# pascalPost/turbomesh

Measured on AMD Instinct MI355X. Metric: nodes smoothed/sec (elliptic sweeps, 4096^2 blocks) + achieved HBM GB/s, higher is better.
Workload: dtype f64

## Files before the change

turbomesh_amd/csrc/tm_kernels.hip:

```cpp
#include "tm_kernels.h"
#include "tm_devutil.hpp"
#include "tm_refmath.h"
#include <cstdlib>
#include <type_traits>

namespace tmh {

__device__ __forceinline__ double lane_prev(double edge, double v) {
    int2 o = __builtin_bit_cast(int2, edge), s = __builtin_bit_cast(int2, v), r;
    r.x = __builtin_amdgcn_update_dpp(o.x, s.x, 0x138 , 0xf, 0xf, false);
    r.y = __builtin_amdgcn_update_dpp(o.y, s.y, 0x138, 0xf, 0xf, false);
    return __builtin_bit_cast(double, r);
}
__device__ __forceinline__ double lane_next(double edge, double v) {
    int2 o = __builtin_bit_cast(int2, edge), s = __builtin_bit_cast(int2, v), r;
    r.x = __builtin_amdgcn_update_dpp(o.x, s.x, 0x130 , 0xf, 0xf, false);
    r.y = __builtin_amdgcn_update_dpp(o.y, s.y, 0x130, 0xf, 0xf, false);
    return __builtin_bit_cast(double, r);
}
__device__ __forceinline__ double2 lane_prev(double2 edge, double2 v) { return make_double2(lane_prev(edge.x, v.x), lane_prev(edge.y, v.y)); }
__device__ __forceinline__ double2 lane_next(double2 edge, double2 v) { return make_double2(lane_next(edge.x, v.x), lane_next(edge.y, v.y)); }

__device__ __forceinline__ double2 lane_prev0(double2 v) {
    int4 s = __builtin_bit_cast(int4, v), r;
// ... 12 lines not shown
    return __builtin_bit_cast(double2, r);
}

enum { S_I_J = 0, S_IP1_J, S_IM1_J, S_I_JP1, S_I_JM1, S_IP1_JP1, S_IP1_JM1, S_IM1_JP1, S_IM1_JM1 };

template <bool HAS_PQ>
__device__ __forceinline__ void stencil_coefs(double2 im1_j, double2 ip1_j, double2 i_jm1, double2 i_jp1, double P, double Q,
                                              double (&c)[9]) {
    const double x_xi = 0.5 * (ip1_j.x - im1_j.x);
    const double x_eta = 0.5 * (i_jp1.x - i_jm1.x);
    const double y_xi = 0.5 * (ip1_j.y - im1_j.y);
    const double y_eta = 0.5 * (i_jp1.y - i_jm1.y);
    const double g22 = x_eta * x_eta + y_eta * y_eta;
    const double g12 = x_xi * x_eta + y_xi * y_eta;
    const double g11 = x_xi * x_xi + y_xi * y_xi;
    c[S_I_J] = -2.0 * g22 - 2.0 * g11;
    if (HAS_PQ) {
        c[S_IP1_J] = g22 * (1 + 0.5 * P);
        c[S_IM1_J] = g22 * (1 - 0.5 * P);
        c[S_I_JP1] = g11 * (1 + 0.5 * Q);
        c[S_I_JM1] = g11 * (1 - 0.5 * Q);
    } else {
        c[S_IP1_J] = g22;
        c[S_IM1_J] = g22;
        c[S_I_JP1] = g11;
        c[S_I_JM1] = g11;
    }
    c[S_IP1_JP1] = -0.5 * g12;
    c[S_IP1_JM1] = 0.5 * g12;
    c[S_IM1_JP1] = 0.5 * g12;
    c[S_IM1_JM1] = -0.5 * g12;
}

template <int MODE>
__device__ __forceinline__ double row_out(double sum, double rhs, double diag, double in_self, double omega) {
    if (MODE == MODE_RAW) return sum;
    const double dinv = (diag == 0.0) ? 1.0 : 1.0 / diag;
    if (MODE == MODE_SCALED) return sum * dinv;
    const double res = rhs * dinv - sum * dinv;
    if (MODE == MODE_RESID) return res;
    return in_self + omega * res;
}

template <int DOT>
__device__ __forceinline__ void accumulate(double (&acc)[MAX_PARTIALS], double2 in_self, double2 out, double2 aux) {
    if (DOT == DOT_AUX) {
        acc[0] += aux.x * out.x;
        acc[1] += aux.y * out.y;
    } else if (DOT == DOT_AUX2) {
        acc[0] += aux.x * out.x;
        acc[1] += aux.y * out.y;
        acc[2] += out.x * out.x;
        acc[3] += out.y * out.y;
    } else if (DOT == DOT_IN) {
        acc[0] += in_self.x * out.x;
        acc[1] += in_self.y * out.y;
        acc[2] += out.x * out.x;
        acc[3] += out.y * out.y;
    } else if (DOT == DOT_IN_SS) {
        acc[0] += in_self.x * out.x;
        acc[1] += in_self.y * out.y;
        acc[2] += out.x * out.x;
        acc[3] += out.y * out.y;
        acc[4] += in_self.x * in_self.x;
        acc[5] += in_self.y * in_self.y;
    } else if (DOT == DOT_B2) {
        acc[0] += in_self.x * out.x;
        acc[1] += in_self.y * out.y;
        acc[2] += out.x * out.x;
        acc[3] += out.y * out.y;
        acc[4] += aux.x * in_self.x;
        acc[5] += aux.y * in_self.y;
        acc[6] += aux.x * out.x;
        acc[7] += aux.y * out.y;
    } else if (DOT == DOT_OUT2) {
        acc[0] += out.x * out.x;
        acc[1] += out.y * out.y;
    } else if (DOT == DOT_DELTA) {
        acc[0] = fma(aux.x, aux.x, acc[0]);
        acc[1] = fma(aux.y, aux.y, acc[1]);
    }
}

__device__ __forceinline__ double recip_diag(double D, double m2D) {
    const bool plain = (D >= 0x1p-700) && (D <= 0x1p700);
    if (__builtin_amdgcn_ballot_w64(!plain) == 0) {
        const double nd = -m2D;
        const double r0 = __builtin_amdgcn_rcp(m2D);
        const double e0 = fma(nd, r0, 1.0);
        const double r1 = fma(r0, e0, r0);
        const double e1 = fma(nd, r1, 1.0);
        const double r2 = fma(r1, e1, r1);
        const double e2 = fma(nd, r2, 1.0);
        return fma(e2, r2, r2);
    }
    return (D == 0.0) ? 0.25 : 1.0 / m2D;
}

template <int MODE, bool HAS_PQ, bool UNIT_OMEGA = false>
__device__ __forceinline__ double2 winslow_row(double2 m_c, double2 e_m, double2 c_c, double2 e_c, double2 h_c, double2 p_c, double2 e_p, double2 dxi,
                                               double2 det, double P, double Q, double omega, double2& delta) {
    const double G11 = fma(dxi.x, dxi.x, dxi.y * dxi.y);
    const double G22 = fma(det.x, det.x, det.y * det.y);
    const double G12 = fma(dxi.x, det.x, dxi.y * det.y);
    const double D = G11 + G22;
    const double m2D = -2.0 * D;
    const double mhG12 = -0.5 * G12;
    double ax = p_c.x + m_c.x, ay = p_c.y + m_c.y;
    double bx = h_c.x, by = h_c.y;
    if (HAS_PQ) {
        const double hP = 0.5 * P, hQ = 0.5 * Q;
        ax = fma(hP, p_c.x - m_c.x, ax);
        ay = fma(hP, p_c.y - m_c.y, ay);
        bx = fma(hQ, e_c.x, bx);
        by = fma(hQ, e_c.y, by);
    }
    const double kx = e_p.x - e_m.x;
    const double ky = e_p.y - e_m.y;
    double sx = G22 * ax, sy = G22 * ay;
    sx = fma(G11, bx, sx);
    sy = fma(G11, by, sy);
    if (MODE == MODE_RELAX && (UNIT_OMEGA || omega == 1.0)) {
        const double qx = fma(mhG12, kx, sx), qy = fma(mhG12, ky, sy);
        const bool plain = (D >= 0x1p-700) && (D <= 0x1p700);
        double2 xn;
        if (__builtin_amdgcn_ballot_w64(!plain) == 0) {
            const double nd = -m2D;
            const double r0 = __builtin_amdgcn_rcp(m2D);
            const double e0 = fma(nd, r0, 1.0);
            const double r1 = fma(r0, e0, r0);
            const double e1 = fma(nd, r1, 1.0);
            const double r2 = fma(r1, e1, r1);
            const double e2 = fma(nd, r2, 1.0);
            const double r = fma(e2, r2, r2);
            xn = make_double2(-(qx * r), -(qy * r));
        } else {
            const double r = 1.0 / m2D;
            xn = (D == 0.0) ? c_c : make_double2(-(qx * r), -(qy * r));
        }
        delta = make_double2(xn.x - c_c.x, xn.y - c_c.y);
        return xn;
    }
    sx = fma(m2D, c_c.x, sx);
    sy = fma(m2D, c_c.y, sy);
    sx = fma(mhG12, kx, sx);
    sy = fma(mhG12, ky, sy);
    if (MODE == MODE_RAW) return make_double2(0.25 * sx, 0.25 * sy);
    const double rinv = recip_diag(D, m2D);
    const double tx = sx * rinv, ty = sy * rinv;
    if (MODE == MODE_SCALED) return make_double2(tx, ty);
    if (MODE == MODE_RESID) return make_double2(-tx, -ty);
    delta = UNIT_OMEGA ? make_double2(-tx, -ty) : make_double2(omega * (-tx), omega * (-ty));
    return make_double2(c_c.x + delta.x, c_c.y + delta.y);
}

__device__ __forceinline__ double2 sub2(double2 a, double2 b) { return make_double2(a.x - b.x, a.y - b.y); }
__device__ __forceinline__ double2 add2(double2 a, double2 b) { return make_double2(a.x + b.x, a.y + b.y); }

template <int NT>
__device__ __forceinline__ const KrylovScalars* lazy_scalars(const LazyScalars& L);

static bool g_rows_forced = false;
static int g_rows_per_chunk = 18;
static int g_unroll = 6;
static int g_nt = 1;

constexpr unsigned OOB_VOFFSET = 0x80000000u;
typedef int v4i32 __attribute__((ext_vector_type(4)));

typedef double d2v __attribute__((ext_vector_type(2)));
__device__ __forceinline__ void store_nt(double2* dst, double2 v) {
    d2v o;
    o.x = v.x;
    o.y = v.y;
    __builtin_nontemporal_store(o, reinterpret_cast<d2v*>(dst));
}

struct VirtualR {
    double2 s, rn, pn;
};
__device__ __forceinline__ VirtualR virtual_r(double2 x, double2 y, double2 z, double2 w, double2 va, double2 vb, double2 vc) {
    VirtualR o;
    o.s = make_double2(x.x - va.x * y.x, x.y - va.y * y.y);
    o.rn = make_double2(o.s.x - vb.x * z.x, o.s.y - vb.y * z.y);
    o.pn = make_double2(o.rn.x + vc.x * (w.x - vb.x * y.x), o.rn.y + vc.y * (w.y - vb.y * y.y));
    return o;
}
template <int VK>
__device__ __forceinline__ double2 virtual_vec(double2 x, double2 y, double2 z, double2 va, double2 vb) {
    if (VK == VK_S || VK == VK_S2) return make_double2(x.x - va.x * y.x, x.y - va.y * y.y);
    if (VK == VK_P) return make_double2(x.x + va.x * (y.x - vb.x * z.x), x.y + va.y * (y.y - vb.y * z.y));
    return x;
}

__device__ __forceinline__ double2 load_nt(const double2* src);

template <int MODE, int DOT, bool FIELD, bool HAS_PQ, int U, bool NT, int VK = VK_NONE, bool OV = false>
__device__ __forceinline__ void apply_tile(const ApplyBlock& a, int RI, int nSG, int nRC, int bid, double2 va = make_double2(0.0, 0.0),
                                           double2 vb = make_double2(0.0, 0.0), double2 vc = make_double2(0.0, 0.0)) {
    static_assert(U % 3 == 0, "the 3-row window rotates by renaming: the row group must be a multiple of 3");
    const int lane = threadIdx.x & 63;
    const int wave = threadIdx.x >> 6;
    const int total = nSG * nRC;
    const int q = total >> 3, rem = total & 7, xcd = bid & 7, k = bid >> 3;
    const int logical = (xcd < rem) ? xcd * (q + 1) + k : rem * (q + 1) + (xcd - rem) * q + k;
    const int rc = logical / nSG;
    const int sg = logical - rc * nSG;

    const int ni = a.ni, nj = a.nj;
    const int j0 = (sg * 4 + wave) * (OV ? 62 : 64);
    const int j = j0 + lane;
    const int jc = min(j, nj - 1);
    const bool edge_lane = !OV && ((lane == 0) || (lane == 63));
    const int hcol = (lane == 0) ? max(j0 - 1, 0) : min(j0 + 64, nj - 1);
    const bool valid_col = (j >= 1) && (j <= nj - 2) && (!OV || (lane >= 1 && lane <= 62));
    const bool full_wave = !OV && (j0 >= 1) && (j0 + 63 <= nj - 2);
    const int i0 = 1 + rc * RI;
    const int i1 = min(i0 + RI, ni - 1);

    double acc[MAX_PARTIALS] = {0.0, 0.0, 0.0, 0.0};
    if ((OV ? (j0 + 1 <= nj - 2) : (j0 < nj)) && i0 < i1) {
// ... 200 lines not shown
                    } else {
                        *dst = o;
                    }
                    if (VK == VK_P) store_nt(a.pout + static_cast<size_t>(row) * nj + j, Wc[C]);
                    accumulate<DOT>(acc, Wc[C], o, (DOT == DOT_AUX || DOT == DOT_AUX2 || DOT == DOT_B2) ? g.auxv[u] : ((DOT == DOT_DELTA) ? delta : o));
                }
                if (!FIELD) Xdet = sub2(lane_next(g.xph[u], g.xpc[u]), lane_prev(g.xph[u], g.xpc[u]));
            }
        };

        int ib = i0;
        if (full_wave) {
            for (; ib + U <= i1; ib += U) {
                Group g;
                load_group(ib, g);
                compute_group(ib, g, std::false_type{});
            }
        }
        for (; ib < i1; ib += U) {
            Group g;
            load_group(ib, g);
            compute_group(ib, g, std::true_type{});
        }
    }
    if ((MODE == MODE_DIAG_NOSTORE || MODE == MODE_DIAG_MATH) && acc[0] + acc[1] == 123.456) a.out[0] = make_double2(acc[0], acc[1]);
    if (DOT != DOT_NONE) block_partials<256, (VK == VK_R ? 4 : dot_columns(DOT))>(acc, a.partials + static_cast<size_t>(bid) * MAX_PARTIALS);
}

template <int MODE, int DOT, bool FIELD, bool HAS_PQ, int U, bool NT>
__global__ __launch_bounds__(256) void k_apply(ApplyBlock a, int RI, int nSG, int nRC) {
    apply_tile<MODE, DOT, FIELD, HAS_PQ, U, NT>(a, RI, nSG, nRC, blockIdx.x);
}

template <int MODE, int DOT, bool FIELD, bool HAS_PQ, int U, bool NT>
__global__ __launch_bounds__(256) void k_apply_batch(ApplyBatch B) {
    int k = 0;
#pragma unroll
    for (int q = 1; q < APPLY_BATCH_MAX; ++q)
        if (q < B.n && static_cast<int>(blockIdx.x) >= B.start[q]) k = q;
    apply_tile<MODE, DOT, FIELD, HAS_PQ, U, NT>(B.b[k], B.RI[k], B.nSG[k], B.nRC[k], static_cast<int>(blockIdx.x) - B.start[k]);
}


template <bool HAS_PQ>
__global__ __launch_bounds__(256) void k_apply_prolong_smooth(ApplyBlock a, int RI, int nSG, int nRC) {
    apply_tile<MODE_MG_SMOOTH, DOT_NONE, false, HAS_PQ, 3, true, VK_PRO>(a, RI, nSG, nRC, blockIdx.x);
}
static inline int rows_per_chunk(int ni, int nj, int rows);
hipError_t launch_mg_prolong_smooth(const ApplyBlock& a0, const MgPair& g, hipStream_t st) {
    if (a0.ni < 3 || a0.nj < 3) return hipSuccess;
    ApplyBlock a = a0;
    a.mg_nic = g.nic;
    a.mg_njc = g.njc;
    a.mg_ci = g.ci;
    a.mg_cj = g.cj;
    const int RI = rows_per_chunk(a.ni, a.nj, a.rows);
    const int nSG = (a.nj + 255) / 256;
    const int nRC = (a.ni - 2 + RI - 1) / RI;
    const dim3 grid(nSG * nRC), block(256);
    if (a.pq) hipLaunchKernelGGL(k_apply_prolong_smooth<true>, grid, block, 0, st, a, RI, nSG, nRC);
    else hipLaunchKernelGGL(k_apply_prolong_smooth<false>, grid, block, 0, st, a, RI, nSG, nRC);
    return hipGetLastError();
}

struct Relax2Tile {
    int c0, c, i0, i1;
    bool out_lane;
};

#ifndef TM_R2_SAUX
#define TM_R2_SAUX 2
#endif
struct Row3 {
    double2 c, e, h;
};
__device__ __forceinline__ Row3 make_row(double2 c) {
    const double2 l = lane_prev0(c), r = lane_next0(c);
    Row3 w;
    w.c = c;
    w.e = sub2(r, l);
    w.h = add2(r, l);
    return w;
}
template <bool W1>
__device__ __forceinline__ double2 relax_row(const Row3& m, const Row3& c, const Row3& p, double omega, double2& delta) {
    return winslow_row<MODE_RELAX, false, W1>(m.c, m.e, c.c, c.e, c.h, p.c, p.e, sub2(p.c, m.c), c.e, 0.0, 0.0, omega, delta);
}

template <int DOT, int U, int NT, bool W1>
__device__ __forceinline__ void relax2_strip_edge(const Relax2Block& a, const Relax2Tile& t, double (&acc)[MAX_PARTIALS]) {
    const int ni = a.ni, nj = a.nj;
    const int cc = min(max(t.c, 0), nj - 1);
    const double2* in_col = a.in + cc;
    const double2* mid_col = a.mid + cc;
    const double2 zero = make_double2(0.0, 0.0);
    auto load_in = [&](int row) { return in_col[static_cast<size_t>(min(max(row, 0), ni - 1)) * nj]; };
    auto load_mid = [&](int row) { return mid_col[static_cast<size_t>(min(max(row, 0), ni - 1)) * nj]; };
    const bool perim_col = (t.c == 0) || (t.c == nj - 1);
    const bool ring_col = (t.c == 1) || (t.c == nj - 2);
    const int nrows = t.i1 - t.i0;
    const __amdgpu_buffer_rsrc_t out_rsrc = __builtin_amdgcn_make_buffer_rsrc(a.out + static_cast<size_t>(t.i0) * nj, 0, nrows * nj * 16, 0x00020000);
    const __amdgpu_buffer_rsrc_t mid_rsrc = __builtin_amdgcn_make_buffer_rsrc(a.mid + static_cast<size_t>(t.i0) * nj, 0, nrows * nj * 16, 0x00020000);
    const unsigned lane_off = static_cast<unsigned>(cc) * 16u;

    Row3 A[3], S[3];
    double2 pa[U], na[U], pm;
    {
        const double2 a0 = load_in(t.i0 - 2), a1 = load_in(t.i0 - 1);
#pragma unroll
        for (int u = 0; u < U; ++u) pa[u] = load_in(t.i0 + u);
        pm = load_mid(t.i0 - 1);
        A[0] = make_row(a0);
        A[1] = make_row(a1);
        A[2].c = A[2].e = A[2].h = zero;
        S[0] = S[1] = S[2] = A[2];
    }
    const int nsteps = nrows + 2;
    auto group = [&](const int tb) {
#pragma unroll
        for (int u = 0; u < U; ++u) na[u] = load_in(t.i0 + tb + U + u);
#pragma unroll
        for (int u = 0; u < U; ++u) {
            const int A0 = u % 3, A1 = (u + 1) % 3, A2 = (u + 2) % 3;
            const int i = t.i0 - 2 + tb + u;
            const int q = i + 1;
            A[A2] = make_row(pa[u]);
            const double2 pm_now = pm;
            pm = load_mid(q + 1);
            double2 d1 = zero;
            double2 s1 = relax_row<W1>(A[A0], A[A1], A[A2], a.omega, d1);
            const bool perim_row = (q <= 0) || (q >= ni - 1);
            if (perim_row || perim_col) s1 = pm_now;
            const bool ring = t.out_lane && !perim_row && (q >= t.i0) && (q < t.i1) && ((q == 1) || (q == ni - 2) || ring_col);
            __builtin_amdgcn_raw_buffer_store_b128(__builtin_bit_cast(v4i32, s1), mid_rsrc,
                                                   static_cast<int>(ring ? lane_off + static_cast<unsigned>((q - t.i0) * nj * 16) : OOB_VOFFSET), 0, 0);
            S[A2] = make_row(s1);
            double2 d2 = zero;
            const double2 o = relax_row<W1>(S[A0], S[A1], S[A2], a.omega, d2);
            const bool live = t.out_lane && (i >= t.i0) && (i < t.i1);
            __builtin_amdgcn_raw_buffer_store_b128(__builtin_bit_cast(v4i32, o), out_rsrc,
                                                   static_cast<int>(live ? lane_off + static_cast<unsigned>((i - t.i0) * nj * 16) : OOB_VOFFSET), 0, (NT & 1) ? TM_R2_SAUX : 0);
            if (DOT == DOT_DELTA) {
                if (!live) d2 = zero;
                accumulate<DOT_DELTA>(acc, S[A1].c, o, d2);
            }
        }
#pragma unroll
        for (int u = 0; u < U; ++u) pa[u] = na[u];
    };
    group(0);
    for (int tb = U; tb < nsteps; tb += U) group(tb);
}

template <int DOT, int U, int NT, bool W1>
__device__ __forceinline__ void relax2_strip_inside(const Relax2Block& a, const Relax2Tile& t, double (&acc)[MAX_PARTIALS]) {
    const int nj = a.nj;
    const double2* in_col = a.in + t.c;
    const int last_row = t.i1 + 1;
    auto load_in = [&](int row) {
        const double2* src = in_col + static_cast<size_t>(min(row, last_row)) * nj;
        return (NT & 2) ? load_nt(src) : *src;
    };
    const __amdgpu_buffer_rsrc_t out_rsrc =
        __builtin_amdgcn_make_buffer_rsrc(a.out + static_cast<size_t>(t.i0) * nj, 0, (t.i1 - t.i0) * nj * 16, 0x00020000);
    const unsigned voff = t.out_lane ? static_cast<unsigned>(t.c) * 16u : OOB_VOFFSET;

// ... 91 lines not shown
    if (subset == R2_BORDER) {
        logical = a.border[bid];
    } else {
        const int q8 = total >> 3, rem = total & 7, xcd = bid & 7, k8 = bid >> 3;
        logical = (xcd < rem) ? xcd * (q8 + 1) + k8 : rem * (q8 + 1) + (xcd - rem) * q8 + k8;
    }
    const int rc = logical / nSG;
    const int sg = logical - rc * nSG;

    const int ni = a.ni, nj = a.nj;
    Relax2Tile t;
    t.c0 = (sg * 4 + wave) * 60;
    t.c = t.c0 - 2 + lane;
    t.out_lane = (lane >= 2) && (lane <= 61) && (t.c >= 1) && (t.c <= nj - 2);
    relax2_chunk_rows(ni, RI, rc, t.i0, t.i1);

    if (subset != R2_ALL && subset != R2_BORDER) {
        const bool wg_inside = !relax2_tile_is_border(ni, nj, t.i0, t.i1, sg, a.dyn);
        const bool mine = wg_inside && (subset == R2_INSIDE || ((subset == R2_INSIDE_A) == (rc < nRC / 2)));
        if (!mine) return;
    }
    double acc[MAX_PARTIALS] = {0.0, 0.0, 0.0, 0.0};
    if (t.c0 <= nj - 2 && t.i0 < t.i1) {
        const bool inside = (t.c0 - 2 >= 2) && (t.c0 + 61 <= nj - 3) && (t.i0 - 2 >= 2) && (t.i1 + 1 <= ni - 3) && ((t.i1 - t.i0) % U == 0);
        if (inside) relax2_strip_inside<DOT, U, NT, W1>(a, t, acc);
        else relax2_strip_edge<DOT, U, NT, W1>(a, t, acc);
    }
    if (DOT != DOT_NONE) block_partials<256, dot_columns(DOT)>(acc, a.partials + static_cast<size_t>(logical) * MAX_PARTIALS);
}

template <int DOT, int U, int NT, bool W1>
__global__ __launch_bounds__(256) void k_relax2(Relax2Block a, int RI, int nSG, int nRC, int subset) {
    relax2_tile<DOT, U, NT, W1>(a, RI, nSG, nRC, subset, blockIdx.x);
}

__device__ __forceinline__ void spin_until(const uint32_t* counter, uint32_t target, uint32_t* error, long long limit_ticks) {
    if (__hip_atomic_load(error, __ATOMIC_RELAXED, __HIP_MEMORY_SCOPE_AGENT) != 0u) return;
    const long long t0 = wall_clock64();
    unsigned polls = 0;
    while (__hip_atomic_load(counter, __ATOMIC_RELAXED, __HIP_MEMORY_SCOPE_AGENT) < target) {
        __builtin_amdgcn_s_sleep(16);
        ++polls;
        if ((polls & 255u) != 0u) continue;
        if (__hip_atomic_load(error, __ATOMIC_RELAXED, __HIP_MEMORY_SCOPE_AGENT) != 0u) break;
        if (wall_clock64() - t0 > limit_ticks) {
            __hip_atomic_store(error, 1u, __ATOMIC_RELAXED, __HIP_MEMORY_SCOPE_AGENT);
            break;
        }
    }
}
__device__ __forceinline__ void queue_wait_in_kernel(const QueueWait& w) {
    if (threadIdx.x == 0) spin_until(w.counter, w.target, w.error, w.limit_ticks);
    __syncthreads();
    __builtin_amdgcn_fence(__ATOMIC_ACQUIRE, "agent");
}
__device__ __forceinline__ void queue_signal_in_kernel(uint32_t* counter) {
    if (counter && blockIdx.x == 0 && threadIdx.x == 0) __hip_atomic_fetch_add(counter, 1u, __ATOMIC_RELEASE, __HIP_MEMORY_SCOPE_AGENT);
}
template <int DOT, int U, int NT, bool W1>
__global__ __launch_bounds__(256) void k_relax2_waited(Relax2Block a, int RI, int nSG, int nRC, int subset, QueueWait w) {
    queue_wait_in_kernel(w);
    relax2_tile<DOT, U, NT, W1>(a, RI, nSG, nRC, subset, blockIdx.x);
}

template <int DOT, int U, int NT, bool W1>
__global__ __launch_bounds__(256) void k_relax2_batch_waited(Relax2Batch B, int subset, QueueWait w) {
    queue_wait_in_kernel(w);
    int k = 0;
#pragma unroll
    for (int q = 1; q < APPLY_BATCH_MAX; ++q)
        if (q < B.n && static_cast<int>(blockIdx.x) >= B.start[q]) k = q;
    relax2_tile<DOT, U, NT, W1>(B.b[k], B.RI[k], B.nSG[k], B.nRC[k], subset, static_cast<int>(blockIdx.x) - B.start[k]);
}
template <int DOT, int U, int NT, bool W1>
__global__ __launch_bounds__(256) void k_relax2_batch(Relax2Batch B, int subset) {
    int k = 0;
#pragma unroll
    for (int q = 1; q < APPLY_BATCH_MAX; ++q)
        if (q < B.n && static_cast<int>(blockIdx.x) >= B.start[q]) k = q;
    relax2_tile<DOT, U, NT, W1>(B.b[k], B.RI[k], B.nSG[k], B.nRC[k], subset, static_cast<int>(blockIdx.x) - B.start[k]);
}

#ifndef TM_R3_WAVES
#define TM_R3_WAVES 1
#endif
constexpr int R3_U = 3;
constexpr int R3_H = 3;
constexpr int R3_W = 64 - 2 * R3_H;
template <int DOT, int U, int NT, bool W1, bool INSIDE>
__device__ __forceinline__ void relax3_strip(const Relax2Block& a, const Relax2Tile& t, double (&acc)[MAX_PARTIALS]) {
    const int ni = a.ni, nj = a.nj;
    const int cc = INSIDE ? t.c : min(max(t.c, 0), nj - 1);
    const double2* in_col = a.in + cc;
    const int last_row = INSIDE ? t.i1 + 2 : ni - 1;
    auto load_in = [&](int row) { return in_col[static_cast<size_t>(INSIDE ? min(row, last_row) : min(max(row, 0), last_row)) * nj]; };
    const bool perim_col = !INSIDE && ((t.c <= 0) || (t.c >= nj - 1));
    const int nrows = t.i1 - t.i0;
    const __amdgpu_buffer_rsrc_t out_rsrc = __builtin_amdgcn_make_buffer_rsrc(a.out + static_cast<size_t>(t.i0) * nj, 0, nrows * nj * 16, 0x00020000);
    const bool skip_col = !INSIDE && (((a.dyn & 4) && t.c <= 2) || ((a.dyn & 8) && t.c >= nj - 3));
    const bool live_lane = t.out_lane && !skip_col;
    const unsigned lane_off = live_lane ? static_cast<unsigned>(cc) * 16u : OOB_VOFFSET;
    const double2 zero = make_double2(0.0, 0.0);

    Row3 A[3], S1[3], S2[3];
    double2 pc[U], pn[U];
    {
        const double2 a0 = load_in(t.i0 - 3), a1 = load_in(t.i0 - 2);
#pragma unroll
        for (int u = 0; u < U; ++u) pc[u] = load_in(t.i0 - 1 + u);
        A[0] = make_row(a0);
        A[1] = make_row(a1);
        A[2].c = A[2].e = A[2].h = zero;
        S1[0] = S1[1] = S1[2] = A[2];
        S2[0] = S2[1] = S2[2] = A[2];
    }
    const int nsteps = nrows + 4;
    auto group = [&](const int tb, const int phase) {
#pragma unroll
        for (int u = 0; u < U; ++u) pn[u] = load_in(t.i0 - 1 + tb + U + u);
#pragma unroll
        for (int u = 0; u < U; ++u) {
            const int A0 = u % 3, A1 = (u + 1) % 3, A2 = (u + 2) % 3;
            const int r = t.i0 - 1 + tb + u;
            A[A2] = make_row(pc[u]);
            double2 d = zero;
            double2 s1 = relax_row<W1>(A[A0], A[A1], A[A2], a.omega, d);
            if (!INSIDE && (perim_col || r - 1 <= 0 || r - 1 >= ni - 1)) s1 = A[A1].c;
            S1[A2] = make_row(s1);
            const bool do2 = phase > 0 || u >= 2, do3 = phase > 1 || (phase == 1 && u >= 1);
            double2 s2 = zero;
            if (do2) {
                s2 = relax_row<W1>(S1[A0], S1[A1], S1[A2], a.omega, d);
                if (!INSIDE && (perim_col || r - 2 <= 0 || r - 2 >= ni - 1)) s2 = S1[A1].c;
            }
            if (do2) S2[A2] = make_row(s2);
            double2 d3 = zero;
            double2 o = zero;
            if (do3) o = relax_row<W1>(S2[A0], S2[A1], S2[A2], a.omega, d3);
            const int i = r - 3;
            const bool row_live = (i >= t.i0) && (i < t.i1) && (INSIDE || !(((a.dyn & 1) && i <= 2) || ((a.dyn & 2) && i >= ni - 3)));
            __builtin_amdgcn_raw_buffer_store_b128(__builtin_bit_cast(v4i32, o), out_rsrc,
                                                   static_cast<int>(row_live ? lane_off + static_cast<unsigned>((i - t.i0) * nj * 16) : OOB_VOFFSET), 0,
                                                   (NT & 1) ? 2 : 0);
            if (DOT == DOT_DELTA) {
                if (!(live_lane && row_live)) d3 = zero;
                accumulate<DOT_DELTA>(acc, S2[A1].c, o, d3);
            }
        }
#pragma unroll
        for (int u = 0; u < U; ++u) pc[u] = pn[u];
    };
    static_assert(U == 3, "the phases below assume three steps per group");
    group(0, 0);
    group(U, 1);
    for (int tb = 2 * U; tb < nsteps; tb += U) group(tb, 2);
}

template <int DOT, int U, int NT, bool W1>
__device__ __forceinline__ void relax3_tile(const Relax2Block& a, int RI, int nSG, int nRC, int bid) {
    const int lane = threadIdx.x & 63;
    const int wave = threadIdx.x >> 6;
    const int total = nSG * nRC;
    const int q8 = total >> 3, rem = total & 7, xcd = bid & 7, k8 = bid >> 3;
    const int logical = (xcd < rem) ? xcd * (q8 + 1) + k8 : rem * (q8 + 1) + (xcd - rem) * q8 + k8;
    const int rc = logical / nSG;
    const int sg = logical - rc * nSG;
    const int ni = a.ni, nj = a.nj;
    Relax2Tile t;
    t.c0 = (sg * 4 + wave) * R3_W;
    t.c = t.c0 - R3_H + lane;
    t.out_lane = (lane >= R3_H) && (lane < 64 - R3_H) && (t.c >= 1) && (t.c <= nj - 2);
    t.i0 = 1 + rc * RI;
    t.i1 = min(t.i0 + RI, ni - 1);
    double acc[MAX_PARTIALS] = {0.0, 0.0, 0.0, 0.0};
    if (t.c0 <= nj - 2 && t.i0 < t.i1) {
        const bool inside = (t.c0 - R3_H >= 1) && (t.c0 - R3_H + 63 <= nj - 2) && (t.i0 - 3 >= 1) && (t.i1 + 2 <= ni - 2);
        if (inside) relax3_strip<DOT, U, NT, W1, true>(a, t, acc);
        else relax3_strip<DOT, U, NT, W1, false>(a, t, acc);
    }
    if (DOT != DOT_NONE) block_partials<256, dot_columns(DOT)>(acc, a.partials + static_cast<size_t>(logical) * MAX_PARTIALS);
}
template <int DOT, int U, int NT, bool W1>
__global__ __launch_bounds__(256, TM_R3_WAVES) void k_relax3(Relax2Block a, int RI, int nSG, int nRC) {
    relax3_tile<DOT, U, NT, W1>(a, RI, nSG, nRC, blockIdx.x);
}
template <int DOT, int U, int NT, bool W1>
__global__ __launch_bounds__(256) void k_relax3_batch(Relax2Batch B) {
    int k = 0;
#pragma unroll
    for (int q = 1; q < APPLY_BATCH_MAX; ++q)
        if (q < B.n && static_cast<int>(blockIdx.x) >= B.start[q]) k = q;
    relax3_tile<DOT, U, NT, W1>(B.b[k], B.RI[k], B.nSG[k], B.nRC[k], static_cast<int>(blockIdx.x) - B.start[k]);
}
static int g_fuse3_rows = 0;
void relax3_rows_for_launch(const int* ni, const int* nj, int n, int* rows, bool beside_chain) {
    static const int forced = [] { const char* e = std::getenv("TM_FUSE3_ROWS"); return e ? std::atoi(e) : 0; }();
    if (forced > 0 || g_fuse3_rows > 0) {
        for (int k = 0; k < n; ++k) rows[k] = std::max(1, std::min(forced > 0 ? forced : g_fuse3_rows, ni[k] - 2));
        return;
    }
    static int slots = 0;
    if (slots == 0) {
        int dev = 0, cus = 0;
        if (hipGetDevice(&dev) != hipSuccess || hipDeviceGetAttribute(&cus, hipDeviceAttributeMultiprocessorCount, dev) != hipSuccess || cus <= 0) cus = 256;
        slots = 3 * cus;
    }
    static const int heights[] = {38, 26, 14, 8};
    const long need = static_cast<long>(slots) * (beside_chain ? 9 : 6);
    int RI = 8;
    for (const int h : heights) {
        long total = 0;
        for (int k = 0; k < n; ++k) {
            const int nstrips = (nj[k] - 1 + R3_W - 1) / R3_W, nSG = (nstrips + 3) / 4, interior = ni[k] - 2, r = std::max(1, std::min(h, interior));
            total += static_cast<long>(nSG) * ((interior + r - 1) / r);
        }
        RI = h;
        if (total * 10 >= need) break;
    }
    for (int k = 0; k < n; ++k) rows[k] = std::max(1, std::min(RI, ni[k] - 2));
}
int relax3_rows_per_chunk(int ni, int nj) {
    int r = 0;
    relax3_rows_for_launch(&ni, &nj, 1, &r, false);
    return r;
}
bool relax3_supported(int ni, int nj) { return ni >= 7 && nj >= 7 && nj <= (1 << 20); }
int relax3_block_nwg(int ni, int nj, int RI) {
    const int nstrips = (nj - 1 + R3_W - 1) / R3_W;
    return ((nstrips + 3) / 4) * ((ni - 2 + RI - 1) / RI);
}
hipError_t launch_relax3_blocks(const Relax2Block* blocks, const int* rows_per_chunk, int n, int dot, hipStream_t st) {
    for (int first = 0; first < n; first += APPLY_BATCH_MAX) {
        Relax2Batch B;
        B.n = 0;
        int total = 0;
        bool w1 = true;
        const bool nts = blocks[first].store_nt != 0;
        for (int k = first; k < n && B.n < APPLY_BATCH_MAX; ++k) {
            const int q = B.n++;
            B.b[q] = blocks[k];
            B.RI[q] = rows_per_chunk[k];
            B.nSG[q] = ((blocks[k].nj - 1 + R3_W - 1) / R3_W + 3) / 4;
            B.nRC[q] = (blocks[k].ni - 2 + B.RI[q] - 1) / B.RI[q];
            B.start[q] = total;
            total += B.nSG[q] * B.nRC[q];
            w1 = w1 && blocks[k].omega == 1.0;
        }
        for (int q = B.n; q < APPLY_BATCH_MAX; ++q) B.start[q] = total;
        if (total == 0) continue;
        const dim3 grid(total), block(256);
#define TM_R3(KERNEL, ...)                                                                                                   \
    do {                                                                                                                     \
        if (dot == DOT_DELTA) {                                                                                              \
            if (w1 && nts) hipLaunchKernelGGL((KERNEL<DOT_DELTA, R3_U, 1, true>), grid, block, 0, st, __VA_ARGS__);          \
            else if (w1) hipLaunchKernelGGL((KERNEL<DOT_DELTA, R3_U, 0, true>), grid, block, 0, st, __VA_ARGS__);            \
            else hipLaunchKernelGGL((KERNEL<DOT_DELTA, R3_U, 1, false>), grid, block, 0, st, __VA_ARGS__);                   \
        } else {                                                                                                             \
            if (w1 && nts) hipLaunchKernelGGL((KERNEL<DOT_NONE, R3_U, 1, true>), grid, block, 0, st, __VA_ARGS__);           \
            else if (w1) hipLaunchKernelGGL((KERNEL<DOT_NONE, R3_U, 0, true>), grid, block, 0, st, __VA_ARGS__);             \
            else hipLaunchKernelGGL((KERNEL<DOT_NONE, R3_U, 1, false>), grid, block, 0, st, __VA_ARGS__);                    \
        }                                                                                                                    \
    } while (0)
        static const bool force_batch = [] { const char* e = std::getenv("TM_R3_FORCE_BATCH"); return e && std::atoi(e) != 0; }();
        if (B.n == 1 && !force_batch) TM_R3(k_relax3, B.b[0], B.RI[0], B.nSG[0], B.nRC[0]);
        else TM_R3(k_relax3_batch, B);
#undef TM_R3
        const hipError_t rc = hipGetLastError();
        if (rc != hipSuccess) return rc;
    }
    return hipSuccess;
// ... 1856 lines not shown
```

turbomesh_amd/configs.py:

```python
from __future__ import annotations

import math

import numpy as np

from . import clustering as cluster
from .boundary import Condition, ConditionTag, Connection, Range, Side
from .discrete import Block2d, Edge, Mesh
from .types import Mat2d


def _default_tfi(i_min, i_max, j_min, j_max):
    return Block2d.init(i_min, i_max, j_min, j_max)


def _seed(i_min: Edge, i_max: Edge, j_min: Edge, j_max: Edge, tfi, snap=True) -> Block2d:
    blk = (tfi or _default_tfi)(i_min, i_max, j_min, j_max)
    if snap:
        d = blk.points.data
        d[:, 0] = i_min.points
        d[:, -1] = i_max.points
        d[0, :] = j_min.points
        d[-1, :] = j_max.points
    return blk


def _uniform_edge(points):
    return Edge(points, cluster.Uniform().compute(len(points)))


def single_block_edges(ni, nj=None, amplitude=0.1):
    nj = nj or ni
    s = cluster.Uniform().compute(ni)
    t = cluster.Uniform().compute(nj)
    a = amplitude
    i_min = np.stack([s, a * np.sin(2 * math.pi * s)], axis=1)
    i_max = np.stack([s, 1.0 - a * np.sin(2 * math.pi * s)], axis=1)
    j_min = np.stack([np.zeros(nj), t], axis=1)
    j_max = np.stack([np.ones(nj), t], axis=1)
    i_min[0], i_min[-1] = (0.0, 0.0), (1.0, 0.0)
    i_max[0], i_max[-1] = (0.0, 1.0), (1.0, 1.0)
    return Edge(i_min, s), Edge(i_max, s.copy()), Edge(j_min, t), Edge(j_max, t.copy())


def single_block(ni, nj=None, amplitude=0.1, tfi=None, perturb=0.0, seed=12345) -> Mesh:
    e = single_block_edges(ni, nj, amplitude)
    blk = _seed(*e, tfi)
    if perturb:
        rng = np.random.default_rng(seed)
        d = blk.points.data
        h = 1.0 / (d.shape[0] - 1)
        d[1:-1, 1:-1] += perturb * h * (rng.random(d[1:-1, 1:-1].shape) - 0.5)
    m = Mesh()
    m.addBlock("block", blk)
    return m


def slices(count, n, first=0, tfi=None, perturb=0.0) -> Mesh:
    m = Mesh()
    for k in range(first, first + count):
        one = single_block(n, n, amplitude=0.05 + 0.001 * k, tfi=tfi, perturb=perturb, seed=12345 + k)
        m.addBlock(f"slice_{k}", one.blocks[0])
    return m


def strip(nblocks, ni, nj=None, amplitude=0.1, tfi=None, reverse_odd=False, only_blocks=None) -> Mesh:
    nj = nj or ni
    t = cluster.Uniform().compute(nj)
    s = cluster.Uniform().compute(ni)

    def curve(k):
        c = np.stack([t, k + amplitude * (1.0 - 2.0 * k / nblocks) * np.sin(2 * math.pi * t)], axis=1)
        c[0], c[-1] = (0.0, float(k)), (1.0, float(k))
        return c

    curves = {k: curve(k) for k in range(nblocks + 1) if only_blocks is None or k in only_blocks or (k - 1) in only_blocks}
    m = Mesh()
    for k in range(nblocks):
        if only_blocks is not None and k not in only_blocks:
            m.addBlock(f"block_{k}", Block2d(Mat2d.placeholder((ni, nj))))
            continue
        left = np.stack([np.zeros(ni), k + s], axis=1)
        right = np.stack([np.ones(ni), k + s], axis=1)
        left[0], left[-1] = curves[k][0], curves[k + 1][0]
        right[0], right[-1] = curves[k][-1], curves[k + 1][-1]
        flip = reverse_odd and (k % 2 == 1)
        if not flip:
            blk = _seed(_uniform_edge(left), _uniform_edge(right), _uniform_edge(curves[k]), _uniform_edge(curves[k + 1]), tfi)
        else:
            blk = _seed(_uniform_edge(right), _uniform_edge(left), _uniform_edge(curves[k][::-1].copy()),
                        _uniform_edge(curves[k + 1][::-1].copy()), tfi)
        m.addBlock(f"block_{k}", blk)
    for k in range(nblocks - 1):
        f0 = reverse_odd and (k % 2 == 1)
        f1 = reverse_odd and ((k + 1) % 2 == 1)
        r0 = Range(k, Side.j_max, nj - 1 if f0 else 0, 0 if f0 else nj - 1)
        r1 = Range(k + 1, Side.j_min, nj - 1 if f1 else 0, 0 if f1 else nj - 1)
        m.connections.append(Connection((r0, r1), None))
    return m


def periodic_channel(ni, nj, pitch=0.8, amplitude=0.08, sliding=True, tfi=None) -> Mesh:
    s = cluster.Uniform().compute(ni)
    t = cluster.Uniform().compute(nj)
    wave = amplitude * np.sin(2 * math.pi * s) * s * (1 - s) * 4
    low = np.stack([s, wave], axis=1)
    up = low.copy()
    up[:, 1] = low[:, 1] + pitch
    inlet = np.stack([np.zeros(nj), low[0, 1] + t * pitch], axis=1)
    outlet = np.stack([1.0 + 0.05 * np.sin(2 * math.pi * t), low[-1, 1] + t * pitch + 0.03 * np.sin(4 * math.pi * t)], axis=1)
    inlet[0], inlet[-1] = low[0], up[0]
    outlet[0], outlet[-1] = low[-1], up[-1]
    m = Mesh()
    m.addBlock("channel", _seed(_uniform_edge(low), _uniform_edge(up), _uniform_edge(inlet), _uniform_edge(outlet), tfi))
    m.connections.append(Connection((Range(0, Side.i_min, 0, ni - 1), Range(0, Side.i_max, 0, ni - 1)), (0.0, pitch)))
    if sliding:
        m.boundary_conditions.append(Condition(Range(0, Side.j_min, 0, nj - 1), ConditionTag.inlet))
    return m


def _warp(xi, eta, a):
    x = xi + a * np.sin(2 * math.pi * eta) * np.cos(0.5 * math.pi * xi)
    y = eta + a * np.sin(2 * math.pi * xi) * (1.0 - 0.5 * eta)
    return np.stack([x, y], axis=1)


def two_by_two(n, m=None, warp=0.04, tfi=None) -> Mesh:
    m_ = m or n
    u = cluster.Uniform().compute(n)
    w = cluster.Uniform().compute(m_)
    xs = [0.0, 0.5, 1.0]
    ys = [0.0, 0.5, 1.0]
    hor = {}
    ver = {}
    for c in range(2):
        for yl in range(3):
            xi = xs[c] + u * 0.5
            hor[(c, yl)] = _warp(xi, np.full(n, ys[yl]), warp)
    for xl in range(3):
        for r in range(2):
            eta = ys[r] + w * 0.5
            ver[(xl, r)] = _warp(np.full(m_, xs[xl]), eta, warp)
    for xl in range(3):
        for yl in range(3):
# ... 47 lines not shown
```

Before: 463.3 billion.

## Restructure relax3 strip: lane-masked stages, ping-pong prefetch, scalar-row loads, per-row store rsrc

Rewrites the fused three-sweep strip kernel. Loads now go through a wave-uniform row base pointer (readfirstlane) plus a per-lane byte offset. Output stores build a per-row buffer resource instead of one large resource indexed by row offset. The prefetch buffers alternate between two arrays, removing the copy loop, and each load is issued inside the per-row step. Each relaxation stage is skipped on lanes whose halo neighbours would be invalid. The reciprocal fast path is computed unconditionally and falls back only when the wave ballot detects extreme diagonals. The intent is to cut VGPR pressure, address arithmetic and wasted halo-lane work, at the cost of more complex control flow and divergent lane masks.

```diff
diff --git a/turbomesh_amd/csrc/tm_kernels.hip b/turbomesh_amd/csrc/tm_kernels.hip
--- a/turbomesh_amd/csrc/tm_kernels.hip
+++ b/turbomesh_amd/csrc/tm_kernels.hip
@@ -118,9 +118,11 @@
     }
 }
 
+#define TM_LIKELY(x) __builtin_expect(!!(x), 1)
+#define TM_UNLIKELY(x) __builtin_expect(!!(x), 0)
 __device__ __forceinline__ double recip_diag(double D, double m2D) {
     const bool plain = (D >= 0x1p-700) && (D <= 0x1p700);
-    if (__builtin_amdgcn_ballot_w64(!plain) == 0) {
+    if (TM_LIKELY(__builtin_amdgcn_ballot_w64(!plain) == 0)) {
         const double nd = -m2D;
         const double r0 = __builtin_amdgcn_rcp(m2D);
         const double e0 = fma(nd, r0, 1.0);
@@ -159,20 +161,18 @@
     if (MODE == MODE_RELAX && (UNIT_OMEGA || omega == 1.0)) {
         const double qx = fma(mhG12, kx, sx), qy = fma(mhG12, ky, sy);
         const bool plain = (D >= 0x1p-700) && (D <= 0x1p700);
-        double2 xn;
-        if (__builtin_amdgcn_ballot_w64(!plain) == 0) {
-            const double nd = -m2D;
-            const double r0 = __builtin_amdgcn_rcp(m2D);
-            const double e0 = fma(nd, r0, 1.0);
-            const double r1 = fma(r0, e0, r0);
-            const double e1 = fma(nd, r1, 1.0);
-            const double r2 = fma(r1, e1, r1);
-            const double e2 = fma(nd, r2, 1.0);
-            const double r = fma(e2, r2, r2);
-            xn = make_double2(-(qx * r), -(qy * r));
-        } else {
-            const double r = 1.0 / m2D;
-            xn = (D == 0.0) ? c_c : make_double2(-(qx * r), -(qy * r));
+        const double nd = -m2D;
+        const double r0 = __builtin_amdgcn_rcp(m2D);
+        const double e0 = fma(nd, r0, 1.0);
+        const double r1 = fma(r0, e0, r0);
+        const double e1 = fma(nd, r1, 1.0);
+        const double r2 = fma(r1, e1, r1);
+        const double e2 = fma(nd, r2, 1.0);
+        const double r = fma(e2, r2, r2);
+        double2 xn = make_double2(-(qx * r), -(qy * r));
+        if (TM_UNLIKELY(__builtin_amdgcn_ballot_w64(!plain) != 0)) {
+            const double rd = 1.0 / m2D;
+            xn = (D == 0.0) ? c_c : make_double2(-(qx * rd), -(qy * rd));
         }
         delta = make_double2(xn.x - c_c.x, xn.y - c_c.y);
         return xn;
@@ -801,27 +801,47 @@
 constexpr int R3_U = 3;
 constexpr int R3_H = 3;
 constexpr int R3_W = 64 - 2 * R3_H;
+typedef __attribute__((address_space(1))) const char global_char;
+__device__ __forceinline__ global_char* uniform_ptr(const char* p) {
+    const uint64_t v = reinterpret_cast<uint64_t>(p);
+    const uint32_t lo = __builtin_amdgcn_readfirstlane(static_cast<uint32_t>(v)), hi = __builtin_amdgcn_readfirstlane(static_cast<uint32_t>(v >> 32));
+    return reinterpret_cast<global_char*>((static_cast<uint64_t>(hi) << 32) | lo);
+}
 template <int DOT, int U, int NT, bool W1, bool INSIDE>
 __device__ __forceinline__ void relax3_strip(const Relax2Block& a, const Relax2Tile& t, double (&acc)[MAX_PARTIALS]) {
     const int ni = a.ni, nj = a.nj;
     const int cc = INSIDE ? t.c : min(max(t.c, 0), nj - 1);
-    const double2* in_col = a.in + cc;
     const int last_row = INSIDE ? t.i1 + 2 : ni - 1;
-    auto load_in = [&](int row) { return in_col[static_cast<size_t>(INSIDE ? min(row, last_row) : min(max(row, 0), last_row)) * nj]; };
+    const unsigned row_bytes = static_cast<unsigned>(nj) * 16u, col_bytes = static_cast<unsigned>(cc) * 16u;
+    const char* in_bytes = reinterpret_cast<const char*>(a.in);
+    unsigned load_off = col_bytes;
+    auto load_in = [&](int row) {
+        const int rr = INSIDE ? min(row, last_row) : min(max(row, 0), last_row);
+        global_char* row_base = uniform_ptr(in_bytes + static_cast<size_t>(rr) * row_bytes);
+        asm volatile("" : "+v"(load_off));
+        const d2v v = *reinterpret_cast<__attribute__((address_space(1))) const d2v*>(row_base + load_off);
+        return make_double2(v.x, v.y);
+    };
     const bool perim_col = !INSIDE && ((t.c <= 0) || (t.c >= nj - 1));
     const int nrows = t.i1 - t.i0;
-    const __amdgpu_buffer_rsrc_t out_rsrc = __builtin_amdgcn_make_buffer_rsrc(a.out + static_cast<size_t>(t.i0) * nj, 0, nrows * nj * 16, 0x00020000);
     const bool skip_col = !INSIDE && (((a.dyn & 4) && t.c <= 2) || ((a.dyn & 8) && t.c >= nj - 3));
     const bool live_lane = t.out_lane && !skip_col;
-    const unsigned lane_off = live_lane ? static_cast<unsigned>(cc) * 16u : OOB_VOFFSET;
+    const unsigned lane_off = live_lane ? col_bytes : OOB_VOFFSET;
+    auto store_row = [&](int i, bool row_live, double2 o) {
+        const __amdgpu_buffer_rsrc_t rsrc =
+            __builtin_amdgcn_make_buffer_rsrc(a.out + static_cast<size_t>(row_live ? i : t.i0) * nj, 0, row_live ? static_cast<int>(row_bytes) : 0, 0x00020000);
+        __builtin_amdgcn_raw_buffer_store_b128(__builtin_bit_cast(v4i32, o), rsrc, static_cast<int>(lane_off), 0, (NT & 1) ? 2 : 0);
+    };
     const double2 zero = make_double2(0.0, 0.0);
+    const int lane = threadIdx.x & 63;
+    const bool m1 = static_cast<unsigned>(lane - 1) < 62u, m2 = static_cast<unsigned>(lane - 2) < 60u, m3 = static_cast<unsigned>(lane - 3) < 58u;
 
     Row3 A[3], S1[3], S2[3];
-    double2 pc[U], pn[U];
+    double2 pa[U], pb[U];
     {
         const double2 a0 = load_in(t.i0 - 3), a1 = load_in(t.i0 - 2);
 #pragma unroll
-        for (int u = 0; u < U; ++u) pc[u] = load_in(t.i0 - 1 + u);
+        for (int u = 0; u < U; ++u) pa[u] = load_in(t.i0 - 1 + u);
         A[0] = make_row(a0);
         A[1] = make_row(a1);
         A[2].c = A[2].e = A[2].h = zero;
@@ -829,45 +849,64 @@
         S2[0] = S2[1] = S2[2] = A[2];
     }
     const int nsteps = nrows + 4;
-    auto group = [&](const int tb, const int phase) {
-#pragma unroll
-        for (int u = 0; u < U; ++u) pn[u] = load_in(t.i0 - 1 + tb + U + u);
+    auto group = [&](const int tb, const int phase, double2 (&pc)[U], double2 (&pn)[U]) {
 #pragma unroll
         for (int u = 0; u < U; ++u) {
             const int A0 = u % 3, A1 = (u + 1) % 3, A2 = (u + 2) % 3;
             const int r = t.i0 - 1 + tb + u;
-            A[A2] = make_row(pc[u]);
-            double2 d = zero;
-            double2 s1 = relax_row<W1>(A[A0], A[A1], A[A2], a.omega, d);
-            if (!INSIDE && (perim_col || r - 1 <= 0 || r - 1 >= ni - 1)) s1 = A[A1].c;
-            S1[A2] = make_row(s1);
+            pn[u] = load_in(r + U);
             const bool do2 = phase > 0 || u >= 2, do3 = phase > 1 || (phase == 1 && u >= 1);
-            double2 s2 = zero;
-            if (do2) {
-                s2 = relax_row<W1>(S1[A0], S1[A1], S1[A2], a.omega, d);
-                if (!INSIDE && (perim_col || r - 2 <= 0 || r - 2 >= ni - 1)) s2 = S1[A1].c;
-            }
-            if (do2) S2[A2] = make_row(s2);
-            double2 d3 = zero;
-            double2 o = zero;
-            if (do3) o = relax_row<W1>(S2[A0], S2[A1], S2[A2], a.omega, d3);
             const int i = r - 3;
             const bool row_live = (i >= t.i0) && (i < t.i1) && (INSIDE || !(((a.dyn & 1) && i <= 2) || ((a.dyn & 2) && i >= ni - 3)));
-            __builtin_amdgcn_raw_buffer_store_b128(__builtin_bit_cast(v4i32, o), out_rsrc,
-                                                   static_cast<int>(row_live ? lane_off + static_cast<unsigned>((i - t.i0) * nj * 16) : OOB_VOFFSET), 0,
-                                                   (NT & 1) ? 2 : 0);
-            if (DOT == DOT_DELTA) {
-                if (!(live_lane && row_live)) d3 = zero;
-                accumulate<DOT_DELTA>(acc, S2[A1].c, o, d3);
+            A[A2].c = pc[u];
+            const double2 l0 = lane_prev0(pc[u]), r0 = lane_next0(pc[u]);
+            double2 l1, r1, l2, r2;
+            if (TM_LIKELY(m1)) {
+                A[A2].e = sub2(r0, l0);
+                A[A2].h = add2(r0, l0);
+                double2 d = zero;
+                double2 s1 = relax_row<W1>(A[A0], A[A1], A[A2], a.omega, d);
+                if (!INSIDE && (perim_col || r - 1 <= 0 || r - 1 >= ni - 1)) s1 = A[A1].c;
+                S1[A2].c = s1;
+                l1 = lane_prev0(s1);
+                r1 = lane_next0(s1);
             }
-        }
-#pragma unroll
-        for (int u = 0; u < U; ++u) pc[u] = pn[u];
+            if (TM_LIKELY(m2)) {
+                S1[A2].e = sub2(r1, l1);
+                S1[A2].h = add2(r1, l1);
+                if (do2) {
+                    double2 d = zero;
+                    double2 s2 = relax_row<W1>(S1[A0], S1[A1], S1[A2], a.omega, d);
+                    if (!INSIDE && (perim_col || r - 2 <= 0 || r - 2 >= ni - 1)) s2 = S1[A1].c;
+                    S2[A2].c = s2;
+                    l2 = lane_prev0(s2);
+                    r2 = lane_next0(s2);
+                }
+            }
+            if (do2 && TM_LIKELY(m3)) {
+                S2[A2].e = sub2(r2, l2);
+                S2[A2].h = add2(r2, l2);
+                if (do3) {
+                    double2 d3 = zero;
+                    const double2 o = relax_row<W1>(S2[A0], S2[A1], S2[A2], a.omega, d3);
+                    store_row(i, row_live, o);
+                    if (DOT == DOT_DELTA) {
+                        if (!(live_lane && row_live)) d3 = zero;
+                        accumulate<DOT_DELTA>(acc, S2[A1].c, o, d3);
+                    }
+                }
+            }
+        }
     };
     static_assert(U == 3, "the phases below assume three steps per group");
-    group(0, 0);
-    group(U, 1);
-    for (int tb = 2 * U; tb < nsteps; tb += U) group(tb, 2);
+    group(0, 0, pa, pb);
+    group(U, 1, pb, pa);
+    int tb = 2 * U;
+    for (; tb + U < nsteps; tb += 2 * U) {
+        group(tb, 2, pa, pb);
+        group(tb + U, 2, pb, pa);
+    }
+    if (tb < nsteps) group(tb, 2, pa, pb);
 }
 
 template <int DOT, int U, int NT, bool W1>
```

Result: no change. 460.0 billion (-0.7%).

## Shrink relax3 wavefront halo using edge-lane halo loads and ping-pong row buffers

Applied to the files above, without the earlier changes.

The fused three-sweep relax kernel now loads the left and right neighbour columns per row through edge lanes, using a buffer resource clamped to the halo rows. This lets the per-wave column halo shrink from three to two, so each wave produces more useful output columns and recomputes less. The prefetch rows now ping-pong between two register arrays instead of being copied at the end of each group. Occupancy hints rise to three waves per SIMD on both the single and batched launches, which may add register pressure or spills. A `slices` config option for non-square blocks is also added.

```diff
diff --git a/turbomesh_amd/configs.py b/turbomesh_amd/configs.py
--- a/turbomesh_amd/configs.py
+++ b/turbomesh_amd/configs.py
@@ -56,10 +56,10 @@
     return m
 
 
-def slices(count, n, first=0, tfi=None, perturb=0.0) -> Mesh:
+def slices(count, n, first=0, tfi=None, perturb=0.0, nj=None) -> Mesh:
     m = Mesh()
     for k in range(first, first + count):
-        one = single_block(n, n, amplitude=0.05 + 0.001 * k, tfi=tfi, perturb=perturb, seed=12345 + k)
+        one = single_block(n, nj or n, amplitude=0.05 + 0.001 * k, tfi=tfi, perturb=perturb, seed=12345 + k)
         m.addBlock(f"slice_{k}", one.blocks[0])
     return m
 
diff --git a/turbomesh_amd/csrc/tm_kernels.hip b/turbomesh_amd/csrc/tm_kernels.hip
--- a/turbomesh_amd/csrc/tm_kernels.hip
+++ b/turbomesh_amd/csrc/tm_kernels.hip
@@ -539,6 +539,14 @@
     w.h = add2(r, l);
     return w;
 }
+__device__ __forceinline__ Row3 make_row(double2 c, double2 hl, double2 hr) {
+    const double2 l = lane_prev(hl, c), r = lane_next(hr, c);
+    Row3 w;
+    w.c = c;
+    w.e = sub2(r, l);
+    w.h = add2(r, l);
+    return w;
+}
 template <bool W1>
 __device__ __forceinline__ double2 relax_row(const Row3& m, const Row3& c, const Row3& p, double omega, double2& delta) {
     return winslow_row<MODE_RELAX, false, W1>(m.c, m.e, c.c, c.e, c.h, p.c, p.e, sub2(p.c, m.c), c.e, 0.0, 0.0, omega, delta);
@@ -796,10 +804,10 @@
 }
 
 #ifndef TM_R3_WAVES
-#define TM_R3_WAVES 1
+#define TM_R3_WAVES 3
 #endif
 constexpr int R3_U = 3;
-constexpr int R3_H = 3;
+constexpr int R3_H = 2;
 constexpr int R3_W = 64 - 2 * R3_H;
 template <int DOT, int U, int NT, bool W1, bool INSIDE>
 __device__ __forceinline__ void relax3_strip(const Relax2Block& a, const Relax2Tile& t, double (&acc)[MAX_PARTIALS]) {
@@ -815,28 +823,45 @@
     const bool live_lane = t.out_lane && !skip_col;
     const unsigned lane_off = live_lane ? static_cast<unsigned>(cc) * 16u : OOB_VOFFSET;
     const double2 zero = make_double2(0.0, 0.0);
+    const int lane = threadIdx.x & 63;
+    const int hrow_lo = INSIDE ? t.i0 - 3 : max(t.i0 - 3, 0), hrow_hi = INSIDE ? t.i1 + 2 : min(t.i1 + 2, ni - 1);
+    const __amdgpu_buffer_rsrc_t in_rsrc =
+        __builtin_amdgcn_make_buffer_rsrc(const_cast<double2*>(a.in) + static_cast<size_t>(hrow_lo) * nj, 0, (hrow_hi - hrow_lo + 1) * nj * 16, 0x00020000);
+    const unsigned hoff_l = (lane == 0) ? static_cast<unsigned>(INSIDE ? t.c - 1 : min(max(t.c - 1, 0), nj - 1)) * 16u : OOB_VOFFSET;
+    const unsigned hoff_r = (lane == 63) ? static_cast<unsigned>(INSIDE ? t.c + 1 : min(max(t.c + 1, 0), nj - 1)) * 16u : OOB_VOFFSET;
+    auto load_halo = [&](unsigned hoff, int row) {
+        const int rr = min(max(row, hrow_lo), hrow_hi) - hrow_lo;
+        return __builtin_bit_cast(double2, __builtin_amdgcn_raw_buffer_load_b128(in_rsrc, static_cast<int>(hoff), rr * nj * 16, 0));
+    };
 
     Row3 A[3], S1[3], S2[3];
-    double2 pc[U], pn[U];
+    double2 pa[U], pb[U], hl[U], hr[U];
     {
         const double2 a0 = load_in(t.i0 - 3), a1 = load_in(t.i0 - 2);
-#pragma unroll
-        for (int u = 0; u < U; ++u) pc[u] = load_in(t.i0 - 1 + u);
-        A[0] = make_row(a0);
-        A[1] = make_row(a1);
+        const double2 l0 = load_halo(hoff_l, t.i0 - 3), r0 = load_halo(hoff_r, t.i0 - 3), l1 = load_halo(hoff_l, t.i0 - 2), r1 = load_halo(hoff_r, t.i0 - 2);
+#pragma unroll
+        for (int u = 0; u < U; ++u) {
+            pa[u] = load_in(t.i0 - 1 + u);
+            hl[u] = load_halo(hoff_l, t.i0 - 1 + u);
+            hr[u] = load_halo(hoff_r, t.i0 - 1 + u);
+        }
+        A[0] = make_row(a0, l0, r0);
+        A[1] = make_row(a1, l1, r1);
         A[2].c = A[2].e = A[2].h = zero;
         S1[0] = S1[1] = S1[2] = A[2];
         S2[0] = S2[1] = S2[2] = A[2];
     }
     const int nsteps = nrows + 4;
-    auto group = [&](const int tb, const int phase) {
+    auto group = [&](const int tb, const int phase, double2 (&pc)[U], double2 (&pn)[U]) {
 #pragma unroll
         for (int u = 0; u < U; ++u) pn[u] = load_in(t.i0 - 1 + tb + U + u);
 #pragma unroll
         for (int u = 0; u < U; ++u) {
             const int A0 = u % 3, A1 = (u + 1) % 3, A2 = (u + 2) % 3;
             const int r = t.i0 - 1 + tb + u;
-            A[A2] = make_row(pc[u]);
+            A[A2] = make_row(pc[u], hl[u], hr[u]);
+            hl[u] = load_halo(hoff_l, r + U);
+            hr[u] = load_halo(hoff_r, r + U);
             double2 d = zero;
             double2 s1 = relax_row<W1>(A[A0], A[A1], A[A2], a.omega, d);
             if (!INSIDE && (perim_col || r - 1 <= 0 || r - 1 >= ni - 1)) s1 = A[A1].c;
@@ -861,13 +886,14 @@
                 accumulate<DOT_DELTA>(acc, S2[A1].c, o, d3);
             }
         }
-#pragma unroll
-        for (int u = 0; u < U; ++u) pc[u] = pn[u];
     };
     static_assert(U == 3, "the phases below assume three steps per group");
-    group(0, 0);
-    group(U, 1);
-    for (int tb = 2 * U; tb < nsteps; tb += U) group(tb, 2);
+    group(0, 0, pa, pb);
+    group(U, 1, pb, pa);
+    for (int tb = 2 * U; tb < nsteps; tb += 2 * U) {
+        group(tb, 2, pa, pb);
+        group(tb + U, 2, pb, pa);
+    }
 }
 
 template <int DOT, int U, int NT, bool W1>
@@ -899,7 +925,7 @@
     relax3_tile<DOT, U, NT, W1>(a, RI, nSG, nRC, blockIdx.x);
 }
 template <int DOT, int U, int NT, bool W1>
-__global__ __launch_bounds__(256) void k_relax3_batch(Relax2Batch B) {
+__global__ __launch_bounds__(256, TM_R3_WAVES) void k_relax3_batch(Relax2Batch B) {
     int k = 0;
 #pragma unroll
     for (int q = 1; q < APPLY_BATCH_MAX; ++q)
```

Result: slower. 450.0 billion before, 439.1 billion after (-2.4%).
